# srinix007/GaussianProcessRegression.jl

Measured on AMD Instinct MI355X. Metric: GP-fit+predict wall-time and K-build GB/s + POTRF TFLOP/s at N=32768, higher is better.
Workload: dtype f64; 1 GPU; C3 fit+posterior: SE+SE+WN, N=32768, d=8, np=8192; N=32768, d=8, np=8192, kernel=SE+SE+WN, nb=128, parallelism=replicas x1

## Files before the change

gaussianprocessregression.jl_amd/csrc/dag.hip:

```cpp
#include <algorithm>
#include <cstdint>

#include "common.hpp"

#ifdef DAG_TRACE
__device__ unsigned long long g_diag_ph[16];
#define DSTAMP_INIT() unsigned long long _dst_t = __builtin_amdgcn_s_memrealtime()
#define DSTAMP(i)                                                   \
  do {                                                              \
    __syncthreads();                                                \
    if (threadIdx.x == 0) {                                         \
      const unsigned long long _t = __builtin_amdgcn_s_memrealtime(); \
      atomicAdd(&g_diag_ph[i], _t - _dst_t);                        \
      if ((i) == 7) atomicAdd(&g_diag_ph[8], 1ull);                 \
      _dst_t = _t;                                                  \
    }                                                               \
  } while (0)
#define DSTAMPW(i)                                                  \
  do {                                                              \
    const unsigned long long _t = __builtin_amdgcn_s_memrealtime(); \
    if (threadIdx.x == 0) atomicAdd(&g_diag_ph[i], _t - _dst_t);    \
    _dst_t = _t;                                                    \
  } while (0)
extern "C" void gpr_debug_diag_phases(unsigned long long* out, int reset) {
  hipMemcpyFromSymbol(out, HIP_SYMBOL(g_diag_ph), sizeof(unsigned long long) * 16);
  if (reset) {
    unsigned long long z[16] = {};
    hipMemcpyToSymbol(HIP_SYMBOL(g_diag_ph), z, sizeof z);
  }
}
#endif

#include "diag_block.hpp"

#ifdef DAG_TRACE
__device__ int g_dag_trace[4096];
#define DTRACE(slot, v)                                                                   \
  do {                                                                                    \
    if (__builtin_amdgcn_readfirstlane(threadIdx.x >> 6) == 0)                            \
      __hip_atomic_store(&g_dag_trace[blockIdx.x * 8 + (slot)], (v), __ATOMIC_RELAXED,     \
                         __HIP_MEMORY_SCOPE_SYSTEM);                                      \
  } while (0)
extern "C" void gpr_debug_dag_trace(int* out, void* stream) {
  hipMemcpyFromSymbolAsync(out, HIP_SYMBOL(g_dag_trace), sizeof(int) * 4096, 0,
                           hipMemcpyDeviceToHost, (hipStream_t)stream);
  hipStreamSynchronize((hipStream_t)stream);
}
#define PROF(var, ...)                                  \
  do {                                                  \
    const unsigned long long _t0 = __builtin_amdgcn_s_memrealtime(); \
    __VA_ARGS__;                                        \
    var += __builtin_amdgcn_s_memrealtime() - _t0;      \
  } while (0)
#else
#define DTRACE(slot, v) \
  do {                  \
  } while (0)
#define PROF(var, ...) \
  do {                 \
    __VA_ARGS__;       \
  } while (0)
#endif

namespace {

constexpr int DT = 128;
constexpr int DTK = 16;
#ifndef DAG_DPB
#define DAG_DPB 4
#endif
constexpr int DPB = DAG_DPB;
constexpr int DSTAGE = (DT + DT) * DTK;
constexpr int DLDS = DPB * DSTAGE;
constexpr int DINT = (DLDS + 2) * 8 <= 160 * 1024 ? DLDS : DLDS - 2;
constexpr int DALLOC = DINT + 2;
constexpr int DNCH = DTK / 2;
constexpr int DRPD = 64 / DNCH;
constexpr int DNDMA = DT / (4 * DRPD);
constexpr int DVM = 2 * DNDMA;
constexpr int DNP = DTK / 8;
static_assert(D2_LDS_QTAIL <= DLDS, "diagonal block must fit in the stage buffers");

typedef double d2 __attribute__((ext_vector_type(2)));

struct DagArgs {
  double* A;
  size_t lda;
  int n, nt;
  double* B;
  size_t ldb;
  int nrhs, ntr;
  double* winv;
  int kglob;
  int* info;
  int* sync;
  int* ustored;
  const unsigned* tasks;
  int ntasks;
  int lower;
  double* G;
  size_t ldg;
  int gbase;
  long long spin_limit;
  int mirror;
  const int* tbatch;
  size_t strA, strB, strW;
  int strS;
};

__device__ __forceinline__ int ld_sc1(const int* p) {
  return __hip_atomic_load(p, __ATOMIC_RELAXED, __HIP_MEMORY_SCOPE_AGENT);
}

template <int VM>
__device__ __forceinline__ void dag_vmcnt() {
  asm volatile("s_waitcnt vmcnt(%0)" ::"n"(VM) : "memory");
}

__device__ __forceinline__ int dag_swz(int row) { return (row >> 1) & 7; }
__device__ __forceinline__ int dag_idx(int row, int chunk) {
  return row * DTK + ((chunk ^ dag_swz(row)) << 1);
}

__device__ __forceinline__ int dag_mblk(int wm, int j) {
  return 4 * (j >> 1) + (wm ? 1 + (j & 1) : 3 * (j & 1));
}

template <bool TRI = false>
__device__ __forceinline__ void dag_accum(d4v (&acc)[4][4], const double* __restrict__ P,
                                          size_t ldp, int mv, const double* __restrict__ Q,
                                          size_t ldq, int nv, int nst, double* lds) {
  if (nst <= 0) return;
  const int tid = threadIdx.x, lane = tid & 63;
  const int w = __builtin_amdgcn_readfirstlane(tid >> 6);
  const int wm = w & 1, wn = w >> 1;
  const double* srcP[DNDMA];
  const double* srcQ[DNDMA];
#pragma unroll
  for (int r = 0; r < DNDMA; ++r) {
    const int row = DRPD * (4 * r + w) + lane / DNCH;
    const int c = (lane % DNCH) ^ dag_swz(row);
    srcP[r] = P + 2 * c + (size_t)min(row, mv - 1) * ldp;
    srcQ[r] = Q + 2 * c + (size_t)min(row, nv - 1) * ldq;
  }
  auto issue = [&](int s) {
    double* base = lds + (s % DPB) * DSTAGE;
    const size_t ko = (size_t)min(s, nst - 1) * DTK;
#pragma unroll
    for (int r = 0; r < DNDMA; ++r) {
      __builtin_amdgcn_global_load_lds(srcP[r] + ko, base + (4 * r + w) * 128, 16, 0, 0);
      __builtin_amdgcn_global_load_lds(srcQ[r] + ko, base + DT * DTK + (4 * r + w) * 128, 16, 0, 0);
    }
  };
  auto read_frags = [&](d2 (&F)[DNP][8], int s) {
    const double* ps = lds + (s % DPB) * DSTAGE;
    const double* qs = ps + DT * DTK;
#pragma unroll
    for (int p = 0; p < DNP; ++p) {
      const int ch = (lane >> 4) + 4 * p;
#pragma unroll
      for (int i = 0; i < 4; ++i)
        F[p][i] = *reinterpret_cast<const d2*>(&qs[dag_idx(wn * 64 + i * 16 + (lane & 15), ch)]);
#pragma unroll
      for (int j = 0; j < 4; ++j) {
        const int mrow = TRI ? 16 * dag_mblk(wm, j) : wm * 64 + j * 16;
        F[p][4 + j] = *reinterpret_cast<const d2*>(&ps[dag_idx(mrow + (lane & 15), ch)]);
      }
    }
  };
  auto mfma_stage = [&](const d2 (&F)[DNP][8], int s) {
    (void)s;
#pragma unroll
    for (int j = 0; j < 4; ++j) {
      if (TRI && dag_mblk(wm, j) < s) continue;
#pragma unroll
      for (int p = 0; p < DNP; ++p)
#pragma unroll
        for (int h = 0; h < 2; ++h)
#pragma unroll
          for (int i = 0; i < 4; ++i)
            acc[i][j] = __builtin_amdgcn_mfma_f64_16x16x4f64(F[p][i][h], F[p][4 + j][h], acc[i][j], 0, 0, 0);
    }
  };
  auto step = [&](int s, d2 (&Fc)[DNP][8], d2 (&Fn)[DNP][8]) {
    __builtin_amdgcn_sched_barrier(0);
    __builtin_amdgcn_s_waitcnt(0xC07F);
    dag_vmcnt<DVM * (DPB - 3)>();
    __builtin_amdgcn_s_barrier();
    issue(s + DPB - 1);
    read_frags(Fn, s + 1);
    mfma_stage(Fc, s);
    if constexpr (TRI) return;
#ifndef DAG_SCHED
#define DAG_SCHED 0
#endif
#if DAG_SCHED == 0
#pragma unroll
    for (int t = 0; t < DVM; ++t) {
      __builtin_amdgcn_sched_group_barrier(0x020, 1, 0);
      __builtin_amdgcn_sched_group_barrier(0x008, 1, 0);
    }
#pragma unroll
    for (int t = 0; t < 8 * DNP; ++t) {
      __builtin_amdgcn_sched_group_barrier(0x100, 1, 0);
      __builtin_amdgcn_sched_group_barrier(0x008, 2, 0);
    }
    __builtin_amdgcn_sched_group_barrier(0x008, 32 * DNP - DVM - 16 * DNP, 0);
#elif DAG_SCHED == 1
#pragma unroll
    for (int t = 0; t < DVM; ++t) {
      __builtin_amdgcn_sched_group_barrier(0x020, 1, 0);
      __builtin_amdgcn_sched_group_barrier(0x008, 2, 0);
    }
#pragma unroll
    for (int t = 0; t < 8 * DNP; ++t) {
      __builtin_amdgcn_sched_group_barrier(0x100, 1, 0);
      __builtin_amdgcn_sched_group_barrier(0x008, 2, 0);
    }
    __builtin_amdgcn_sched_group_barrier(0x008, 32 * DNP - 2 * DVM - 16 * DNP, 0);
#elif DAG_SCHED == 2
#pragma unroll
    for (int t = 0; t < 8 * DNP; ++t) {
      __builtin_amdgcn_sched_group_barrier(0x100, 1, 0);
      __builtin_amdgcn_sched_group_barrier(0x008, 1, 0);
    }
#pragma unroll
    for (int t = 0; t < DVM; ++t) {
      __builtin_amdgcn_sched_group_barrier(0x020, 1, 0);
      __builtin_amdgcn_sched_group_barrier(0x008, 2, 0);
    }
    __builtin_amdgcn_sched_group_barrier(0x008, 32 * DNP - 2 * DVM - 8 * DNP, 0);
#endif
  };
  d2 F0[DNP][8], F1[DNP][8];
#pragma unroll
  for (int t = 0; t < DPB - 1; ++t) issue(t);
  dag_vmcnt<DVM * (DPB - 2)>();
  __builtin_amdgcn_s_barrier();
  read_frags(F0, 0);
  __builtin_amdgcn_s_waitcnt(0xC07F);
  int s = 0;
  for (; s + 1 < nst; s += 2) {
    step(s, F0, F1);
    step(s + 1, F1, F0);
  }
  if (s < nst) mfma_stage(F0, s);
  dag_vmcnt<0>();
  __syncthreads();
}


__device__ __forceinline__ int dag_wait(const int* pa, const int* pb, int have, int cap,
                                        int* info, long long limit, int* sh) {
  if (__builtin_amdgcn_readfirstlane(threadIdx.x >> 6) == 0) {
    int v = 0;
    long long spins = 0;
    for (;;) {
      v = __builtin_amdgcn_readfirstlane(min(ld_sc1(pa), ld_sc1(pb)));
      if (v > have) break;
      if (++spins > limit) {
        atomicCAS(info, 0, -1);
        v = cap;
        break;
      }
      __builtin_amdgcn_s_sleep(2);
    }
    *sh = min(v, cap);
  }
  __builtin_amdgcn_fence(__ATOMIC_ACQUIRE, "workgroup");
  __syncthreads();
  const int r = __builtin_amdgcn_readfirstlane(*sh);
  __syncthreads();
  return r;
}

__device__ __forceinline__ void dag_publish(int* prog, int v) {
  asm volatile("s_waitcnt vmcnt(0)" ::: "memory");
  __syncthreads();
  if (__builtin_amdgcn_readfirstlane(threadIdx.x >> 6) == 0)
    __hip_atomic_store(prog, v, __ATOMIC_RELAXED, __HIP_MEMORY_SCOPE_AGENT);
}

__device__ __attribute__((noinline)) int dag_factor(double* S, int mv, int kglob, double* winv) {
  lds_d* L = (lds_d*)S;
  lds_d(*Xd)[D2_PB] = reinterpret_cast<lds_d(*)[D2_PB]>(L + D2_PK);
  lds_i* fail = reinterpret_cast<lds_i*>(L + D2_PK + 4 * D2_PB);
  return diag2_core<true, true>(L, Xd, fail, nullptr, 0, mv, kglob, winv);
}

__device__ __attribute__((noinline)) void dag_store_u(const double* S, double* T, size_t lda, int mv,
                                                      bool sc1) {
  const lds_d* L = (const lds_d*)S;
  if (sc1)
    diag2_store_u<true>(L, T, lda, mv);
  else
    diag2_store_u<false>(L, T, lda, mv);
}

__device__ __forceinline__ void dag_gram_task(const DagArgs& a, int i_, int j_,
                                                        double* lds, int* s_wait,
                                                        unsigned long long& p_wait,
                                                        unsigned long long& p_acc) {
  (void)p_wait;
  (void)p_acc;
  const int i = __builtin_amdgcn_readfirstlane(i_), j = __builtin_amdgcn_readfirstlane(j_);
  const int n = __builtin_amdgcn_readfirstlane(a.n), nt = __builtin_amdgcn_readfirstlane(a.nt);
  const int tid = threadIdx.x, lane = tid & 63;
  const int w = __builtin_amdgcn_readfirstlane(tid >> 6);
  const int wm = w & 1, wn = w >> 1;
  const int* rhsprog = a.sync + 2 + nt;
  double* T = a.G + (size_t)i * DT + (size_t)j * DT * a.ldg;
  const int mv = min(DT, n - i * DT), nv = min(DT, n - j * DT);
  d4v acc[4][4];
#pragma unroll
  for (int ii = 0; ii < 4; ++ii)
#pragma unroll
    for (int jj = 0; jj < 4; ++jj) acc[ii][jj] = d4v{0.0, 0.0, 0.0, 0.0};
  const double* Pcol = a.B + (size_t)i * DT * a.ldb;
  const double* Qcol = a.B + (size_t)j * DT * a.ldb;
  int done = j;
  while (done < nt) {
    int r = 0;
    PROF(p_wait, r = dag_wait(rhsprog + i, rhsprog + j, done, nt, a.info, a.spin_limit, s_wait));
    const int nst = (min(r * DT, n) - done * DT) / DTK;
    PROF(p_acc, dag_accum(acc, Pcol + (size_t)done * DT, a.ldb, mv, Qcol + (size_t)done * DT, a.ldb,
                          nv, nst, lds));
    done = r;
  }
#pragma unroll
  for (int ii = 0; ii < 4; ++ii)
#pragma unroll
    for (int r = 0; r < 4; ++r) {
      const int nn = wn * 64 + ii * 16 + (lane >> 4) + 4 * r;
#pragma unroll
      for (int jj = 0; jj < 4; ++jj) {
        const int mm = wm * 64 + jj * 16 + (lane & 15);
        if (mm < mv && nn < nv && (i != j || mm <= nn))
          T[(size_t)mm + (size_t)nn * a.ldg] = acc[ii][jj][r];
      }
    }
  double* Tm = a.G + (size_t)j * DT + (size_t)i * DT * a.ldg;
#pragma unroll
  for (int ii = 0; ii < 4; ++ii)
#pragma unroll
    for (int jj = 0; jj < 4; ++jj)
#pragma unroll
      for (int r = 0; r < 4; ++r) {
        const int nn = wn * 64 + ii * 16 + (lane >> 4) + 4 * r;
        const int mm = wm * 64 + jj * 16 + (lane & 15);
        if (mm < mv && nn < nv && (i != j || mm < nn))
          Tm[(size_t)nn + (size_t)mm * a.ldg] = acc[ii][jj][r];
      }
}

template <bool GRAM, bool BATCH>
__global__ __launch_bounds__(256, 1) void potrf_dag_kernel(DagArgs a0) {
  DagArgs a = a0;
  __shared__ double lds[DALLOC];
  int& s_task = reinterpret_cast<int*>(lds + DINT)[0];
  int& s_skip = reinterpret_cast<int*>(lds + DINT)[1];
  int& s_wait = reinterpret_cast<int*>(lds + DINT)[2];
  int s_fok = 0;
  const int tid = threadIdx.x, lane = tid & 63;
  const int w = __builtin_amdgcn_readfirstlane(tid >> 6);
  const int wm = w & 1, wn = w >> 1;
  int* colprog = a.sync + 2;
  int* rhsprog = colprog + a.nt;
  unsigned long long p_wait = 0, p_acc = 0, p_fac = 0, p_tri = 0, p_all = 0, p_n = 0;
#ifdef DAG_PROF_PUB
  unsigned long long p_pub = 0, p_tri_unused = 0;
#define p_tri p_tri_unused
#endif
  (void)p_wait; (void)p_acc; (void)p_fac; (void)p_tri; (void)p_all; (void)p_n;
#ifdef DAG_TRACE
  const unsigned long long p_start = __builtin_amdgcn_s_memrealtime();
#endif
  for (;;) {
    if (w == 0) {
      const int tk = atomicAdd(&a0.sync[0], lane == 0 ? 1 : 0);
      const int tk0 = __builtin_amdgcn_readlane(tk, 0);
      s_task = tk0;
      if (!BATCH) {
        s_skip = __builtin_amdgcn_readfirstlane(ld_sc1(a.info)) != 0;
      } else if (tk0 < a0.ntasks) {
        const int b = __builtin_amdgcn_readfirstlane(a0.tbatch[tk0]);
        s_skip = __builtin_amdgcn_readfirstlane(ld_sc1(a0.info + b)) != 0;
      }
    }
    __syncthreads();
    const int t = __builtin_amdgcn_readfirstlane(s_task);
    const bool skip = __builtin_amdgcn_readfirstlane(s_skip);
    DTRACE(0, t);
    DTRACE(1, 1);
    if (t >= a.ntasks) break;
    if (BATCH) {
      const int b = __builtin_amdgcn_readfirstlane(a0.tbatch[t]);
      a.A = a0.A + (size_t)b * a0.strA;
      a.B = a0.B + (size_t)b * a0.strB;
      a.winv = a0.winv + (size_t)b * a0.strW;
      a.info = a0.info + b;
      colprog = a0.sync + (size_t)b * a0.strS + 2;
      rhsprog = colprog + a.nt;
    }
    const unsigned code = __builtin_amdgcn_readfirstlane(a.tasks[t]);
    if (GRAM && t >= a.gbase) {
      if (!skip) dag_gram_task(a, (code >> 16) & 0x7fff, code & 0xffff, lds, &s_wait, p_wait, p_acc);
      ++p_n;
      __syncthreads();
      continue;
    }
    const bool rhs = code >> 31;
    const int i = (code >> 16) & 0x7fff, j = code & 0xffff;
    const bool diag = !rhs && i == j;
    double* T = rhs ? a.B + (size_t)i * DT + (size_t)j * DT * a.ldb
                    : a.A + (size_t)i * DT + (size_t)j * DT * a.lda;
    const size_t ldt = rhs ? a.ldb : a.lda;
    const double* Qcol = rhs ? a.B + (size_t)j * DT * a.ldb : a.A + (size_t)j * DT * a.lda;
    const double* Pcol = a.A + (size_t)i * DT * a.lda;
    int* pj = rhs ? rhsprog + j : colprog + j;
    const int mv = min(DT, a.n - i * DT);
    const int nv = min(DT, (rhs ? a.nrhs : a.n) - j * DT);
    if (!skip) {
      d4v acc[4][4];
#pragma unroll
      for (int ii = 0; ii < 4; ++ii)
#pragma unroll
        for (int r = 0; r < 4; ++r) {
          const int nn = wn * 64 + ii * 16 + (lane >> 4) + 4 * r;
          const double* col = T + (size_t)min(nn, nv - 1) * ldt;
#pragma unroll
          for (int jj = 0; jj < 4; ++jj) {
            const int mm = wm * 64 + jj * 16 + (lane & 15);
            const double c = col[min(mm, mv - 1)];
            acc[ii][jj][r] = (mm < mv && nn < nv) ? -c : 0.0;
          }
        }
      if (a.mirror && !rhs && !diag) {
        double* Tm = a.A + (size_t)j * DT + (size_t)i * DT * a.lda;
#pragma unroll
        for (int ii = 0; ii < 4; ++ii)
#pragma unroll
          for (int jj = 0; jj < 4; ++jj)
#pragma unroll
            for (int r = 0; r < 4; ++r) {
              const int nn = wn * 64 + ii * 16 + (lane >> 4) + 4 * r;
              const int mm = wm * 64 + jj * 16 + (lane & 15);
              if (mm < mv && nn < nv) Tm[(size_t)nn + (size_t)mm * a.lda] = -acc[ii][jj][r];
            }
      }
      DTRACE(1, 2);
      int done = (rhs && a.lower) ? j : 0;
      while (done < i) {
        int r = 0;
        PROF(p_wait, r = dag_wait(colprog + i, pj, done, i, a.info, a.spin_limit, &s_wait));
        PROF(p_acc, dag_accum(acc, Pcol + (size_t)done * DT, a.lda, mv, Qcol + (size_t)done * DT,
                              ldt, nv, (r - done) * (DT / DTK), lds));
        done = r;
      }
      if (diag) {
        double* S = lds;
#pragma unroll
        for (int ii = 0; ii < 4; ++ii)
#pragma unroll
          for (int r = 0; r < 4; ++r) {
            const int nn = wn * 64 + ii * 16 + (lane >> 4) + 4 * r;
#pragma unroll
            for (int jj = 0; jj < 4; ++jj) {
              const int mm = wm * 64 + jj * 16 + (lane & 15);
              if (mm <= nn) S[pk(mm, nn)] = nn < mv ? -acc[ii][jj][r] : (mm == nn ? 1.0 : 0.0);
            }
          }
        __syncthreads();
        DTRACE(1, 3);
        int f = 0;
        PROF(p_fac, f = dag_factor(S, mv, a.kglob + i * DT, a.winv + (size_t)i * DT * DT));
        if (f && w == 0) atomicCAS(a.info, 0, f);
        s_fok = f == 0;
        DTRACE(1, 4);
      } else {
        if (i > 0) {
#pragma unroll
          for (int ii = 0; ii < 4; ++ii)
#pragma unroll
            for (int r = 0; r < 4; ++r) {
              const int nn = wn * 64 + ii * 16 + (lane >> 4) + 4 * r;
#pragma unroll
              for (int jj = 0; jj < 4; ++jj) {
                const int mm = wm * 64 + jj * 16 + (lane & 15);
                if (mm < mv && nn < nv) T[(size_t)mm + (size_t)nn * ldt] = -acc[ii][jj][r];
              }
            }
        }
        asm volatile("s_waitcnt vmcnt(0)" ::: "memory");
        __builtin_amdgcn_fence(__ATOMIC_RELEASE, "workgroup");
        PROF(p_wait, dag_wait(colprog + i, colprog + i, i, i + 1, a.info, a.spin_limit, &s_wait));
#pragma unroll
        for (int ii = 0; ii < 4; ++ii)
#pragma unroll
          for (int jj = 0; jj < 4; ++jj) acc[ii][jj] = d4v{0.0, 0.0, 0.0, 0.0};
        const bool tri = mv == DT;
        if (tri)
          PROF(p_tri, dag_accum<true>(acc, a.winv + (size_t)i * DT * DT, DT, mv, T, ldt, nv, DT / DTK, lds));
        else
          PROF(p_tri, dag_accum(acc, a.winv + (size_t)i * DT * DT, DT, mv, T, ldt, nv, mv / DTK, lds));
#pragma unroll
        for (int ii = 0; ii < 4; ++ii)
#pragma unroll
          for (int r = 0; r < 4; ++r) {
            const int nn = wn * 64 + ii * 16 + (lane >> 4) + 4 * r;
#pragma unroll
            for (int jj = 0; jj < 4; ++jj) {
              const int mm = (tri ? 16 * dag_mblk(wm, jj) : wm * 64 + jj * 16) + (lane & 15);
              if (mm < mv && nn < nv) st_res<true>(&T[(size_t)mm + (size_t)nn * ldt], acc[ii][jj][r]);
            }
          }
      }
    } else if (a.mirror && !rhs && !diag) {
      double* Tm = a.A + (size_t)j * DT + (size_t)i * DT * a.lda;
      for (int e = tid; e < DT * DT; e += 256) {
        const int mm = e & (DT - 1), nn = e >> 7;
        if (mm < mv && nn < nv) Tm[(size_t)nn + (size_t)mm * a.lda] = T[(size_t)mm + (size_t)nn * ldt];
      }
    }
    DTRACE(1, 5);
#ifdef DAG_PROF_PUB
    if (diag) PROF(p_pub, dag_publish(pj, i + 1)); else dag_publish(pj, i + 1);
#else
    dag_publish(pj, i + 1);
#endif
    DTRACE(1, 6);
    if (diag && !skip && __builtin_amdgcn_readfirstlane(s_fok))
      dag_store_u(lds, T, a.lda, mv, a.ustored != nullptr);
    if (diag && a.ustored) dag_publish(a.ustored + i, 1);
    ++p_n;
  }
  DTRACE(1, 7);
#ifdef DAG_TRACE
  p_all = __builtin_amdgcn_s_memrealtime() - p_start;
  DTRACE(2, (int)p_wait);
  DTRACE(3, (int)p_acc);
  DTRACE(4, (int)p_fac);
#ifdef DAG_PROF_PUB
#undef p_tri
  DTRACE(5, (int)p_pub);
  (void)p_tri_unused;
#else
  DTRACE(5, (int)p_tri);
#endif
  DTRACE(6, (int)p_all);
  DTRACE(7, (int)p_n);
#endif
}

}

__global__ void dag_init_kernel(int* sync, int nt, int ntr, int solve, int lower) {
  for (int t = blockIdx.x * blockDim.x + threadIdx.x; t < nt + ntr; t += gridDim.x * blockDim.x)
    sync[2 + t] = t < nt ? (solve ? t + 1 : 0) : (lower ? t - nt : 0);
}

static long long dag_spin_limit(const gpr_ctx* ctx) {
#ifdef GPR_TESTING
  if (const char* sl = getenv("GPR_DAG_SPIN_LIMIT")) return std::max(1ll, atoll(sl));
#endif
  return ctx->dag_spin_limit;
}

bool dag_shape_ok(int n, int lda, const double* dA) {
  return n > 0 && n % 16 == 0 && lda % 16 == 0 && ((uintptr_t)dA & 127) == 0 && n <= DT * 32767;
}

bool dag_takes_whole(const gpr_ctx* ctx, int n, int lda, const double* dA) {
  (void)lda;
  (void)dA;
  return ctx->dag_mode && ctx->nb == DT && n > 0 &&
         n <= DT * 32767 - 16;
}

__global__ void dag_pad_in_kernel(const double* __restrict__ A, size_t lda, int n,
                                  double* __restrict__ W, int n2) {
  const size_t tot = (size_t)n2 * n2;
  for (size_t t = blockIdx.x * (size_t)blockDim.x + threadIdx.x; t < tot;
       t += (size_t)gridDim.x * blockDim.x) {
    const int r = (int)(t % n2), c = (int)(t / n2);
    if (r <= c) W[t] = c < n ? A[(size_t)r + (size_t)c * lda] : (r == c ? 1.0 : 0.0);
  }
}

__global__ void dag_pad_out_kernel(double* __restrict__ A, size_t lda, int n,
                                   const double* __restrict__ W, int n2) {
  const size_t tot = (size_t)n * n;
  for (size_t t = blockIdx.x * (size_t)blockDim.x + threadIdx.x; t < tot;
       t += (size_t)gridDim.x * blockDim.x) {
    const int r = (int)(t % n), c = (int)(t / n);
    if (r <= c) A[(size_t)r + (size_t)c * lda] = W[(size_t)r + (size_t)c * n2];
  }
}

int launch_potrf_dag_padded(gpr_ctx* ctx, double* dA, int n, int lda, double* dB, int nrhs,
                            int ldb) {
  const int n2 = (n + 15) / 16 * 16;
  hipStream_t st = ctx->stream;
  if (ensure_buf(ctx, &ctx->dpadA, &ctx->padA_cap, (size_t)n2 * n2) != 0 ||
      (dB && ensure_buf(ctx, &ctx->dpadB, &ctx->padB_cap, (size_t)n2 * nrhs) != 0)) {
    ctx->err.clear();
    (void)hipGetLastError();
    return 1;
  }
  const int blocks = 2048;
  dag_pad_in_kernel<<<blocks, 256, 0, st>>>(dA, (size_t)lda, n, ctx->dpadA, n2);
  LAUNCH_CHECK(ctx);
  if (dB) {
    HIP_TRY(ctx, hipMemcpy2DAsync(ctx->dpadB, (size_t)n2 * sizeof(double), dB,
                                  (size_t)ldb * sizeof(double), (size_t)n * sizeof(double), nrhs,
                                  hipMemcpyDeviceToDevice, st));
    if (n2 > n)
      HIP_TRY(ctx, hipMemset2DAsync(ctx->dpadB + n, (size_t)n2 * sizeof(double), 0,
                                    (size_t)(n2 - n) * sizeof(double), nrhs, st));
  }
  const int rc = launch_potrf_dag(ctx, ctx->dpadA, n2, n2, dB ? ctx->dpadB : nullptr, nrhs, n2, 0,
                                  st, 0);
  if (rc) return rc < 0 ? rc : set_err(ctx, GPR_E_HIP, "padded tile-DAG: shape not eligible");
  dag_pad_out_kernel<<<blocks, 256, 0, st>>>(dA, (size_t)lda, n, ctx->dpadA, n2);
  LAUNCH_CHECK(ctx);
  if (dB)
    HIP_TRY(ctx, hipMemcpy2DAsync(dB, (size_t)ldb * sizeof(double), ctx->dpadB,
                                  (size_t)n2 * sizeof(double), (size_t)n * sizeof(double), nrhs,
                                  hipMemcpyDeviceToDevice, st));
  return 0;
}

int launch_potrf_dag(gpr_ctx* ctx, double* dA, int n, int lda, double* dB, int nrhs, int ldb,
                     int kglob, hipStream_t st, int flags, double* dG, int ldg) {
  const bool solve = flags & DAG_SOLVE, lower = flags & DAG_LOWER, gram = flags & DAG_GRAM;
  const bool mirror = flags & DAG_MIRROR;
  if ((solve || lower) && (!dB || kglob)) return 1;
  if (mirror && (solve || kglob)) return 1;
  if (gram && (!lower || !dG || ldg < n || nrhs != n)) return 1;
  if (ctx->nb != DT || n <= 0 || n % 16 || lda % 16 || ((uintptr_t)dA & 127) || n > DT * 32767 ||
      kglob % DT)
    return 1;
  if (dB && (nrhs <= 0 || ldb % 16 || ((uintptr_t)dB & 127) || nrhs > DT * 65535)) return 1;
  const int nt = (n + DT - 1) / DT, ntr = dB ? (nrhs + DT - 1) / DT : 0;
  GPR_TRY(ensure_winv(ctx, kglob + n, DT));
  if (ctx->dag_nt != nt || ctx->dag_ntr != ntr || ctx->dag_flags != (flags & ~DAG_MIRROR) ||
      ctx->dag_lag_built != ctx->dag_zlag) {
    std::vector<unsigned> tasks;
    tasks.reserve((size_t)nt * (nt + 1) + (size_t)nt * ntr);
    const int lag = solve || !lower ? 0 : std::min(ctx->dag_zlag, nt);
    auto rhs_row = [&](int i) {
      for (int c = 0; c < (lower ? std::min(ntr, i + 1) : ntr); ++c)
        tasks.push_back(0x80000000u | ((unsigned)i << 16) | (unsigned)c);
    };
    for (int i = 0; i < nt; ++i) {
      if (!solve)
        for (int j = i; j < nt; ++j) tasks.push_back(((unsigned)i << 16) | (unsigned)j);
      if (i - lag >= 0) rhs_row(i - lag);
    }
    for (int i = std::max(nt - lag, 0); i < nt; ++i) rhs_row(i);
    if (gram)
      for (int j = 0; j < nt; ++j)
        for (int i = 0; i <= j; ++i) tasks.push_back(((unsigned)i << 16) | (unsigned)j);
    if (ctx->dag_tasks) {
      HIP_TRY(ctx, hipStreamSynchronize(ctx->stream));
      HIP_TRY(ctx, hipFree(ctx->dag_tasks));
    }
    ctx->dag_tasks = nullptr;
    ctx->dag_nt = ctx->dag_ntr = -1;
    HIP_TRY(ctx, hipMalloc((void**)&ctx->dag_tasks, tasks.size() * sizeof(unsigned)));
    HIP_TRY(ctx, hipMemcpy(ctx->dag_tasks, tasks.data(), tasks.size() * sizeof(unsigned),
                           hipMemcpyHostToDevice));
    ctx->dag_ntasks = (int)tasks.size();
    ctx->dag_nt = nt;
    ctx->dag_ntr = ntr;
    ctx->dag_flags = flags & ~DAG_MIRROR;
    ctx->dag_lag_built = ctx->dag_zlag;
  }
  if (ctx->dag_sync_readers_pending) {
    HIP_TRY(ctx, hipStreamWaitEvent(st, ctx->dag_sync_readers, 0));
    HIP_TRY(ctx, hipStreamWaitEvent(ctx->stream, ctx->dag_sync_readers, 0));
    ctx->dag_sync_readers_pending = false;
  }
  const size_t nsync = 2 + (size_t)nt + ntr + nt;
  if (ctx->dag_sync_cap < nsync) {
    if (ctx->dag_sync) {
      HIP_TRY(ctx, hipStreamSynchronize(ctx->stream));
      HIP_TRY(ctx, hipFree(ctx->dag_sync));
    }
    ctx->dag_sync = nullptr;
    ctx->dag_sync_cap = 0;
    HIP_TRY(ctx, hipMalloc((void**)&ctx->dag_sync, nsync * sizeof(int)));
    ctx->dag_sync_cap = nsync;
  }
  HIP_TRY(ctx, hipMemsetAsync(ctx->dag_sync, 0, nsync * sizeof(int), st));
  if (solve || lower) {
    dag_init_kernel<<<(nt + ntr + 255) / 256, 256, 0, st>>>(ctx->dag_sync, nt, ntr, solve, lower);
    LAUNCH_CHECK(ctx);
  }
  if (ctx->ncu <= 0) {
    hipDeviceProp_t prop;
    HIP_TRY(ctx, hipGetDeviceProperties(&prop, ctx->device));
    ctx->ncu = prop.multiProcessorCount;
  }
  DagArgs a{};
  a.A = dA;
  a.lda = (size_t)lda;
  a.n = n;
  a.nt = nt;
  a.B = dB;
  a.ldb = (size_t)(dB ? ldb : 0);
  a.nrhs = dB ? nrhs : 0;
  a.ntr = ntr;
  a.winv = ctx->winv + (size_t)(kglob / DT) * DT * DT;
  a.kglob = kglob;
  a.info = ctx->dinfo;
  a.sync = ctx->dag_sync;
  a.tasks = ctx->dag_tasks;
  a.ntasks = ctx->dag_ntasks;
  a.lower = lower;
  a.G = gram ? dG : nullptr;
  a.ldg = (size_t)(gram ? ldg : 0);
  a.gbase = gram ? ctx->dag_ntasks - nt * (nt + 1) / 2 : ctx->dag_ntasks;
  a.mirror = mirror;
  a.spin_limit = dag_spin_limit(ctx);
  const int grid = std::min(ctx->dag_ntasks, std::max(1, ctx->ncu - ctx->dag_reserve_cu));
  auto hook = (ctx->dag_hook && !solve && !lower && kglob == 0) ? ctx->dag_hook : nullptr;
  a.ustored = hook ? ctx->dag_sync + 2 + nt + ntr : nullptr;
  hipEvent_t hook_ev = nullptr;
  if (hook) {
    ctx->dag_hook = nullptr;
    if (hipEventCreateWithFlags(&hook_ev, hipEventDisableTiming) != hipSuccess) hook_ev = nullptr;
    if (hook_ev && hipEventRecord(hook_ev, st) != hipSuccess) {
      hipEventDestroy(hook_ev);
      hook_ev = nullptr;
    }
    (void)hipGetLastError();
  }
  const double flops = (solve ? 0.0 : (double)n * n * n / 3.0) +
                       (lower ? (double)n * n * n / 3.0 : (double)n * n * (dB ? nrhs : 0)) +
                       (gram ? (double)n * n * n / 3.0 : 0.0);
  {
    hipStream_t ls = ctx->ls;
    ctx->ls = st;
    TimerScope ts(ctx, solve ? TC_DAG_SOLVE : TC_DAG, flops);
    if (gram)
      potrf_dag_kernel<true, false><<<grid, 256, 0, st>>>(a);
    else
      potrf_dag_kernel<false, false><<<grid, 256, 0, st>>>(a);
    ctx->ls = ls;
    const hipError_t le = hipGetLastError();
    if (le != hipSuccess) {
      if (hook_ev) hipEventDestroy(hook_ev);
      return set_err(ctx, GPR_E_HIP, "tile-DAG launch: %s", hipGetErrorString(le));
    }
  }
  if (hook) {
    hook(ctx->dag_hook_user, dA, n, lda, ctx->dag_sync + 2, a.ustored, nt, hook_ev);
    if (hook_ev) hipEventDestroy(hook_ev);
  }
  return 0;
}

int launch_potrf_dag_batch(gpr_ctx* ctx, double* dA, size_t strA, int n, int lda, double* dB,
                           size_t strB, int nrhs, int ldb, int nbatch, int* info_out) {
  hipStream_t st = ctx->stream;
  if (nbatch <= 0) return 0;
  if (n <= 0 || n % 16 || lda % 16 || strA % 16 || ((uintptr_t)dA & 127) || n > DT * 32767)
    return 1;
  if (dB && (nrhs <= 0 || ldb % 16 || strB % 16 || ((uintptr_t)dB & 127) || nrhs > DT * 65535))
    return 1;
  const int nt = (n + DT - 1) / DT, ntr = dB ? (nrhs + DT - 1) / DT : 0;
  std::vector<unsigned> tasks;
  std::vector<int> tb;
  const size_t per = (size_t)nt * (nt + 1) / 2 + (size_t)nt * ntr;
  tasks.reserve(per * nbatch);
  tb.reserve(per * nbatch);
  for (int i = 0; i < nt; ++i) {
    for (int b = 0; b < nbatch; ++b)
      for (int j = i; j < nt; ++j) {
        tasks.push_back(((unsigned)i << 16) | (unsigned)j);
        tb.push_back(b);
      }
    for (int b = 0; b < nbatch; ++b)
      for (int c = 0; c < ntr; ++c) {
        tasks.push_back(0x80000000u | ((unsigned)i << 16) | (unsigned)c);
        tb.push_back(b);
      }
  }
  const int ntasks = (int)tasks.size();
  const int strS = 2 + nt + ntr;
  const size_t nW = (size_t)nbatch * nt * DT * DT;
  const size_t nI = (size_t)ntasks * 2 + (size_t)nbatch * strS + (size_t)nbatch;
  GPR_TRY(ensure_buf(ctx, &ctx->dagb, &ctx->dagb_cap, nW + (nI + 1) / 2 + 1));
  double* W = ctx->dagb;
  unsigned* dtasks = reinterpret_cast<unsigned*>(W + nW);
  int* dtb = reinterpret_cast<int*>(dtasks + ntasks);
  int* dsync = dtb + ntasks;
  int* dinfo = dsync + (size_t)nbatch * strS;
  HIP_TRY(ctx, hipMemcpyAsync(dtasks, tasks.data(), sizeof(unsigned) * ntasks, hipMemcpyHostToDevice, st));
  HIP_TRY(ctx, hipMemcpyAsync(dtb, tb.data(), sizeof(int) * ntasks, hipMemcpyHostToDevice, st));
  HIP_TRY(ctx, hipMemsetAsync(dsync, 0, sizeof(int) * ((size_t)nbatch * strS + nbatch), st));
  if (ctx->ncu <= 0) {
    hipDeviceProp_t prop;
    HIP_TRY(ctx, hipGetDeviceProperties(&prop, ctx->device));
    ctx->ncu = prop.multiProcessorCount;
  }
  DagArgs a{};
  a.A = dA;
  a.lda = (size_t)lda;
  a.n = n;
  a.nt = nt;
  a.B = dB;
  a.ldb = (size_t)(dB ? ldb : 0);
  a.nrhs = dB ? nrhs : 0;
  a.ntr = ntr;
  a.winv = W;
  a.kglob = 0;
  a.info = dinfo;
  a.sync = dsync;
  a.tasks = dtasks;
  a.ntasks = ntasks;
  a.gbase = ntasks;
  a.spin_limit = dag_spin_limit(ctx);
  a.tbatch = dtb;
  a.strA = strA;
  a.strB = strB;
  a.strW = (size_t)nt * DT * DT;
  a.strS = strS;
  const int grid = std::min(ntasks, std::max(1, ctx->ncu));
  const double flops = nbatch * ((double)n * n * n / 3.0 + (double)n * n * (dB ? nrhs : 0));
  {
    TimerScope ts(ctx, TC_DAG, flops);
    potrf_dag_kernel<false, true><<<grid, 256, 0, st>>>(a);
    const hipError_t le = hipGetLastError();
    if (le != hipSuccess) return set_err(ctx, GPR_E_HIP, "batched tile-DAG launch: %s", hipGetErrorString(le));
  }
  std::vector<int> h(nbatch);
  HIP_TRY(ctx, hipMemcpyAsync(h.data(), dinfo, sizeof(int) * nbatch, hipMemcpyDeviceToHost, st));
  HIP_TRY(ctx, hipStreamSynchronize(st));
  for (int b = 0; b < nbatch; ++b) {
    if (h[b] < 0) return set_err(ctx, GPR_E_HIP, "batched tile-DAG: a dependency wait timed out");
    if (info_out) info_out[b] = h[b];
  }
  return 0;
}
```

Measured before the change: 3.206 GP jobs/s (fit N=32768 + posterior mean/var np=8192, per GPU).

## Deepen DAG GEMM LDS pipeline to five stages with one barrier per two steps

The default number of LDS stages in dag_accum goes from 4 to 5. A new unrolled 'period' loop processes two k-steps per LDS barrier, using explicit ring-buffer indices in place of modulo arithmetic, and uses its own sched_group_barrier interleaving of MFMA, DS reads and global-to-LDS loads. The goal is to halve the barrier and waitcnt stalls per k-step and keep more global loads in flight. The cost is that the stage buffers now take nearly the whole 160KB of LDS, which limits occupancy and leaves almost no room for anything else in LDS. The buffer-reuse safety also depends on the two-step ordering.

```diff
diff --git a/gaussianprocessregression.jl_amd/csrc/dag.hip b/gaussianprocessregression.jl_amd/csrc/dag.hip
--- a/gaussianprocessregression.jl_amd/csrc/dag.hip
+++ b/gaussianprocessregression.jl_amd/csrc/dag.hip
@@ -67,8 +67,9 @@
 constexpr int DT = 128;
 constexpr int DTK = 16;
 #ifndef DAG_DPB
-#define DAG_DPB 4
-#endif
+#define DAG_DPB 5
+#endif
+static_assert(DAG_DPB == 4 || DAG_DPB == 5, "dag_accum is written for 4 or 5 LDS stages");
 constexpr int DPB = DAG_DPB;
 constexpr int DSTAGE = (DT + DT) * DTK;
 constexpr int DLDS = DPB * DSTAGE;
@@ -143,8 +144,8 @@
     srcP[r] = P + 2 * c + (size_t)min(row, mv - 1) * ldp;
     srcQ[r] = Q + 2 * c + (size_t)min(row, nv - 1) * ldq;
   }
-  auto issue = [&](int s) {
-    double* base = lds + (s % DPB) * DSTAGE;
+  auto issue = [&](int s, int b) {
+    double* base = lds + b * DSTAGE;
     const size_t ko = (size_t)min(s, nst - 1) * DTK;
 #pragma unroll
     for (int r = 0; r < DNDMA; ++r) {
@@ -152,8 +153,8 @@
       __builtin_amdgcn_global_load_lds(srcQ[r] + ko, base + DT * DTK + (4 * r + w) * 128, 16, 0, 0);
     }
   };
-  auto read_frags = [&](d2 (&F)[DNP][8], int s) {
-    const double* ps = lds + (s % DPB) * DSTAGE;
+  auto read_frags = [&](d2 (&F)[DNP][8], int b) {
+    const double* ps = lds + b * DSTAGE;
     const double* qs = ps + DT * DTK;
 #pragma unroll
     for (int p = 0; p < DNP; ++p) {
@@ -182,13 +183,64 @@
             acc[i][j] = __builtin_amdgcn_mfma_f64_16x16x4f64(F[p][i][h], F[p][4 + j][h], acc[i][j], 0, 0, 0);
     }
   };
+#if DAG_DPB == 5
+  d2 F0[DNP][8], F1[DNP][8];
+  auto ring = [](int b, int k) { return b + k >= DPB ? b + k - DPB : b + k; };
+  auto period = [&](int s, int b) {
+    __builtin_amdgcn_sched_barrier(0);
+    __builtin_amdgcn_s_waitcnt(0xC07F);
+    dag_vmcnt<DVM>();
+    __builtin_amdgcn_s_barrier();
+    issue(s + 4, ring(b, 4));
+    read_frags(F1, ring(b, 1));
+    mfma_stage(F0, s);
+    if constexpr (!TRI) {
+      __builtin_amdgcn_sched_group_barrier(0x008, 1, 0);
+#pragma unroll
+      for (int t = 0; t < DVM; ++t) {
+        __builtin_amdgcn_sched_group_barrier(0x020, 1, 0);
+        __builtin_amdgcn_sched_group_barrier(0x008, 2, 0);
+      }
+#pragma unroll
+      for (int t = 0; t < 8 * DNP; ++t) {
+        __builtin_amdgcn_sched_group_barrier(0x100, 1, 0);
+        __builtin_amdgcn_sched_group_barrier(0x008, 2, 0);
+      }
+      __builtin_amdgcn_sched_group_barrier(0x008, 32 * DNP - 1 - 2 * DVM - 16 * DNP, 0);
+    }
+    issue(s + 5, b);
+    read_frags(F0, ring(b, 2));
+    mfma_stage(F1, s + 1);
+    if constexpr (!TRI) {
+#pragma unroll
+      for (int t = 0; t < DVM; ++t) {
+        __builtin_amdgcn_sched_group_barrier(0x020, 1, 0);
+        __builtin_amdgcn_sched_group_barrier(0x008, 2, 0);
+      }
+#pragma unroll
+      for (int t = 0; t < 8 * DNP; ++t) {
+        __builtin_amdgcn_sched_group_barrier(0x100, 1, 0);
+        __builtin_amdgcn_sched_group_barrier(0x008, 2, 0);
+      }
+      __builtin_amdgcn_sched_group_barrier(0x008, 32 * DNP - 2 * DVM - 16 * DNP, 0);
+    }
+  };
+#pragma unroll
+  for (int t = 0; t < DPB - 1; ++t) issue(t, t);
+  dag_vmcnt<DVM * (DPB - 2)>();
+  __builtin_amdgcn_s_barrier();
+  read_frags(F0, 0);
+  __builtin_amdgcn_s_waitcnt(0xC07F);
+  int s = 0;
+  for (int b = 0; s + 1 < nst; s += 2, b = ring(b, 2)) period(s, b);
+#else
   auto step = [&](int s, d2 (&Fc)[DNP][8], d2 (&Fn)[DNP][8]) {
     __builtin_amdgcn_sched_barrier(0);
     __builtin_amdgcn_s_waitcnt(0xC07F);
     dag_vmcnt<DVM * (DPB - 3)>();
     __builtin_amdgcn_s_barrier();
-    issue(s + DPB - 1);
-    read_frags(Fn, s + 1);
+    issue(s + DPB - 1, (s + DPB - 1) % DPB);
+    read_frags(Fn, (s + 1) % DPB);
     mfma_stage(Fc, s);
     if constexpr (TRI) return;
 #ifndef DAG_SCHED
@@ -234,7 +286,7 @@
   };
   d2 F0[DNP][8], F1[DNP][8];
 #pragma unroll
-  for (int t = 0; t < DPB - 1; ++t) issue(t);
+  for (int t = 0; t < DPB - 1; ++t) issue(t, t);
   dag_vmcnt<DVM * (DPB - 2)>();
   __builtin_amdgcn_s_barrier();
   read_frags(F0, 0);
@@ -244,6 +296,7 @@
     step(s, F0, F1);
     step(s + 1, F1, F0);
   }
+#endif
   if (s < nst) mfma_stage(F0, s);
   dag_vmcnt<0>();
   __syncthreads();
```

Measured after the change: 3.243 GP jobs/s (fit N=32768 + posterior mean/var np=8192, per GPU) (median of 6 runs). 1.2% higher.
